# Srecharan/Leaf-Grasping-Vision-ML

Hardware: AMD Instinct MI355X
Metric: frames/sec (1080p depth+mask) grasp scoring, 1/8 MI355X; % HBM roofline (higher is better)
Workload: dtype f32; 1 GPU; 1080x1920 depth+mask, 8 score planes + valid + top-20 NMS + GraspPointCNN fp32 rescoring of 20 candidates; height=1080, width=1920, batches_in_flight=1, parallelism=frames sharded over 1 GPU(s), no collective

## Files before the change

### include/leafgrasp.h

```cpp
#ifndef LEAFGRASP_H
#define LEAFGRASP_H

#include <stdint.h>

#ifdef __cplusplus
extern "C" {
#endif

typedef struct lg_ctx* lg_handle;

typedef enum lg_status {
    LG_OK = 0,
    LG_ERR_INVALID = -1,
    LG_ERR_HIP = -2,
    LG_ERR_NOMEM = -3,
    LG_ERR_NO_MODEL = -4,
    LG_ERR_UNSUPPORTED = -5,
    LG_ERR_BUSY = -6
} lg_status;

enum {
    LG_MAP_SDF = 0,
    LG_MAP_APPROACH = 1,
    LG_MAP_FLATNESS = 2,
// ... 200 lines not shown

int lg_debug_dt_max(lg_handle h, int frame, uint32_t out[2], int32_t win[4]);
int lg_debug_dt_form(lg_handle h, int frame, int32_t form[2]);
int lg_debug_dt_search_form(lg_handle h, int32_t* algo);
int lg_dt_form_host(int forced, int n, int H, int W);
int lg_debug_orient_redo(lg_handle h, int32_t* n);
int lg_near_tile_rect(int bx0, int bx1, int by0, int by1, int H, int W, int halo, int32_t rect[4]);
int lg_stem_words_host(const uint64_t* bits, int H, int W, int WW, int bottom_start, int k, uint64_t* out);
int lg_stem_words_host_spans(const uint64_t* bits, int H, int W, int WW, int bottom_start, int n, int anchor, const int8_t* lo,
                             const int8_t* hi, int algo, uint64_t* out);
int lg_stem_plan(int k, int n, int anchor, const int8_t* lo, const int8_t* hi, int32_t* i0, int8_t span_lo[64], int8_t span_hi[64],
                 int8_t dlo[64], int8_t dhi[64]);
int lg_window_from_box(const uint32_t box[5], int H, int W, int search_mode, int32_t out[12]);
int lg_border_line_max(const int32_t* prof, int n, int lo, int len, uint32_t* out);
int lg_debug_near_tiles(lg_handle h, int32_t* off, int cap);
int lg_options_text(int which, char* buf, int cap);
int lg_debug_options(lg_handle h, char* buf, int cap);
int lg_debug_cnn_scored(lg_handle h, int64_t* patches);
int lg_debug_leaf_fallback(lg_handle h, int32_t* flags, int cap, int32_t* n_frames, int32_t* n_flagged);
int lg_debug_cnn_survivors(lg_handle h, int32_t* sub_frames, int32_t* n_sub, int32_t* counts, int32_t counts_cap,
                           int32_t* list, int32_t* slot, float* logits, int64_t cap, int64_t* n_slots);
int lg_debug_patch(lg_handle h, int64_t slot, float* out);
int lg_debug_isolation_fields(lg_handle h, int frame, uint32_t* dc_fix, uint32_t* dw_fix, uint32_t max_fix[2]);
int lg_label_aware_check(const lg_params* p, int has_labels);
int lg_norm3_host(const int32_t* dx, const int32_t* dy, int n, uint32_t* out);
int lg_dilate_words_host(const uint64_t* bits, int H, int W, int WW, int k, uint64_t* out);
int lg_debug_ws_plane_bytes(lg_handle h, int64_t bytes[LG_NUM_MAPS]);
int lg_wave_rows_on_mask(const uint64_t* bits, int H, int WW, int y, int w);

typedef struct lg_trainer lg_trainer;
// ... 46 lines not shown
```

### leaf-grasping-vision-ml_amd/_lib.py

```python
import ctypes as C
import os

_HERE = os.path.dirname(os.path.abspath(__file__))
LIB_PATH = os.environ.get("LG_LIB_PATH") or os.path.join(_HERE, "liblgrasp.so")

LG_NUM_MAPS = 8
MAP_NAMES = ("sdf_score", "approach_score", "flatness_map", "isolation_map", "distance_map",
             "accessibility_map", "stem_penalty", "traditional_score")
MAP_INDEX = {n: i for i, n in enumerate(MAP_NAMES)}

LG_OK, LG_ERR_INVALID, LG_ERR_HIP, LG_ERR_NOMEM, LG_ERR_NO_MODEL, LG_ERR_UNSUPPORTED, LG_ERR_BUSY = 0, -1, -2, -3, -4, -5, -6


class LgParams(C.Structure):
    _fields_ = [(n, C.c_double) for n in ("cx", "cy", "f")] + [(n, C.c_float) for n in (
        "w_approach", "w_sdf", "w_flat", "w_access", "sdf_w_interior", "sdf_w_align",
        "sdf_w_sdf", "optimal_distance", "access_w_dist", "access_w_dir", "flat_scale", "iso_w_close",
        "iso_w_wide", "iso_ramp_top", "iso_ramp_bottom", "min_edge_distance", "stem_valid_thresh")] + \
        [(n, C.c_int32) for n in ("stem_se", "stem_bottom_div", "top_k", "nms_min_distance",
                                  "pregrasp_clearance", "mask_is_bool", "gaussian_size", "chamfer_init_dist0", "label_aware")]


_FP = C.POINTER(C.c_float)

# ... 124 lines not shown
    "lg_debug_dt_form": (C.c_int, [_VP, C.c_int, C.POINTER(C.c_int32)]),
    "lg_debug_orient_redo": (C.c_int, [_VP, C.POINTER(C.c_int32)]),
    "lg_options_text": (C.c_int, [C.c_int, C.c_char_p, C.c_int]),
    "lg_debug_options": (C.c_int, [_VP, C.c_char_p, C.c_int]),
    "lg_debug_dt_search_form": (C.c_int, [_VP, C.POINTER(C.c_int32)]),
    "lg_dt_form_host": (C.c_int, [C.c_int, C.c_int, C.c_int, C.c_int]),
    "lg_near_tile_rect": (C.c_int, [C.c_int, C.c_int, C.c_int, C.c_int, C.c_int, C.c_int, C.c_int, C.POINTER(C.c_int32)]),
    "lg_stem_words_host": (C.c_int, [_VP, C.c_int, C.c_int, C.c_int, C.c_int, C.c_int, _VP]),
    "lg_stem_words_host_spans": (C.c_int, [_VP, C.c_int, C.c_int, C.c_int, C.c_int, C.c_int, C.c_int, C.POINTER(C.c_int8),
                                           C.POINTER(C.c_int8), C.c_int, _VP]),
    "lg_stem_plan": (C.c_int, [C.c_int, C.c_int, C.c_int, C.POINTER(C.c_int8), C.POINTER(C.c_int8), C.POINTER(C.c_int32),
                               C.POINTER(C.c_int8), C.POINTER(C.c_int8), C.POINTER(C.c_int8), C.POINTER(C.c_int8)]),
    "lg_window_from_box": (C.c_int, [C.POINTER(C.c_uint32), C.c_int, C.c_int, C.c_int, C.POINTER(C.c_int32)]),
    "lg_border_line_max": (C.c_int, [C.POINTER(C.c_int32), C.c_int, C.c_int, C.c_int, C.POINTER(C.c_uint32)]),
    "lg_debug_near_tiles":(C.c_int, [_VP, C.POINTER(C.c_int32), C.c_int]),
    "lg_debug_cnn_scored": (C.c_int, [_VP, C.POINTER(C.c_int64)]),
    "lg_debug_leaf_fallback": (C.c_int, [_VP, C.POINTER(C.c_int32), C.c_int, C.POINTER(C.c_int32), C.POINTER(C.c_int32)]),
    "lg_debug_cnn_survivors": (C.c_int, [_VP, C.POINTER(C.c_int32), C.POINTER(C.c_int32), C.POINTER(C.c_int32), C.c_int32,
                                         C.POINTER(C.c_int32), C.POINTER(C.c_int32), _FP, C.c_int64, C.POINTER(C.c_int64)]),
    "lg_debug_patch": (C.c_int, [_VP, C.c_int64, _FP]),
    "lg_debug_isolation_fields": (C.c_int, [_VP, C.c_int, _VP, _VP, C.POINTER(C.c_uint32)]),
    "lg_label_aware_check": (C.c_int, [C.POINTER(LgParams), C.c_int]),
    "lg_norm3_host": (C.c_int, [_VP, _VP, C.c_int, _VP]),
    "lg_dilate_words_host": (C.c_int, [_VP, C.c_int, C.c_int, C.c_int, C.c_int, _VP]),
    "lg_debug_ws_plane_bytes": (C.c_int, [_VP, C.POINTER(C.c_int64)]),
    "lg_wave_rows_on_mask": (C.c_int, [_VP, C.c_int, C.c_int, C.c_int, C.c_int]),
    "lg_harvest_patches": (C.c_int, [_VP, _VP, _VP, _VP, C.c_int, C.c_int, C.c_int, _VP, _VP, _VP, _VP, _VP, _VP, _VP]),
    "lg_negative_masks": (C.c_int, [_VP, _VP, _VP, C.c_int, C.c_int, _VP, _VP, _VP]),
    "lg_leaf_contour": (C.c_int, [_VP, _VP, C.c_int, C.c_int, _VP, C.c_int, C.POINTER(C.c_int), _VP]),
    "lg_train_create": (C.c_int, [C.c_int, C.c_int, C.POINTER(C.c_int32), C.c_int, C.c_int, C.POINTER(_VP)]),
# ... 58 lines not shown
```

### leaf-grasping-vision-ml_amd/csrc/lg_cnn.h

```cpp
#pragma once
#include <hip/hip_runtime.h>

#include <string>

#include "../../include/leafgrasp.h"

struct RtLayer { int cin, cout, cinp, coutp, wi; bool pool; };

struct LgCnnPlan {
    int n_layers = 6;
    RtLayer layers[8] = {};
    bool standard = true;
    int F = 256, Fp = 256, npix = 16;
    size_t act_per_patch = 64 * 32 * 32;
    int hid = 16;
    int dims[5] = {256, 256, 128, 64, 1};
};
int lg_cnn_plan(int n_blocks, const int32_t* filters, int attention_type, bool need_head, LgCnnPlan* p, std::string* err);
bool wino_supported(int cin, int cout, int wi, bool pool);
bool lg_head_supported(int F, int npix);

struct LgCnn : LgCnnPlan {
    bool loaded = false;
    float* wconv[8] = {nullptr};
// ... 14 lines not shown
    size_t act_per[8] = {0};
    float* in_halo = nullptr;
    float* zeros = nullptr;
    float* kpart = nullptr;
    unsigned* kflag = nullptr;
    unsigned* kerr_host = nullptr;
    unsigned* kerr_dev = nullptr;
    int wino_mask = 0x3f;
    int capN = 0;
    long long weight_allocs = 0;
};

int lg_cnn_upload(LgCnn* c, const lg_cnn_weights* w, std::string* err);
void lg_cnn_free(LgCnn* c);
int lg_cnn_run(LgCnn* c, const float* patches, bool haloed_in, int N, float* logits, hipStream_t s, std::string* err,
               bool allow_split = true, const int* n_dev = nullptr);
bool lg_cnn_counts_on_device(const LgCnn* c);
size_t lg_cnn_halo_patch_floats(void);
bool lg_cnn_take_error(LgCnn* c);

struct LgTrainView {
    int device = 0, n_blocks = 0, att = 0, F = 0, hid = 0;
    int filters[4] = {0, 0, 0, 0};
    float bn_eps = 1e-5f;
    const float* P = nullptr;
    const float* B = nullptr;
    size_t conv_w[8] = {0}, conv_b[8] = {0}, bn_g[8] = {0}, bn_b[8] = {0};
    size_t bn_m[8] = {0}, bn_v[8] = {0};
    size_t att_w = 0, att_b = 0, ca_w1 = 0, ca_b1 = 0, ca_w2 = 0, ca_b2 = 0;
    size_t fc_w[4] = {0}, fc_b[4] = {0}, fbn_g[3] = {0}, fbn_b[3] = {0};
    size_t fbn_m[3] = {0}, fbn_v[3] = {0};
// ... 6 lines not shown
```

### leaf-grasping-vision-ml_amd/csrc/lg_cnn.hip

```cpp
#include "lg_cnn.h"

#include <math.h>

#include <algorithm>
#include <type_traits>

typedef float f32x16 __attribute__((ext_vector_type(16)));

#ifndef LG_W4_S0
#define LG_W4_S0 9
#define LG_W4_S1 0
#define LG_W4_S2 0
#define LG_W4_S3 0
#define LG_W4_S4 3
#endif
#ifndef LG_W4_NT
#define LG_W4_NT 0
#endif
#ifndef LG_W4_EXP
#define LG_W4_EXP 0
#endif

namespace {

// ... 1163 lines not shown
        c->act_per[L] = per;
        ok = hipMalloc((void**)&c->act[L], (size_t)N * per * sizeof(float)) == hipSuccess &&
             hipMemsetAsync(c->act[L], 0, (size_t)N * per * sizeof(float), s) == hipSuccess;
    }
    ok = ok && hipMalloc((void**)&c->in_halo, (size_t)N * lg_cnn_halo_patch_floats() * sizeof(float)) == hipSuccess &&
         hipMemsetAsync(c->in_halo, 0, (size_t)N * lg_cnn_halo_patch_floats() * sizeof(float), s) == hipSuccess;
    if (!ok) {
        *err = "lg_cnn_forward: activation workspace allocation failed";
        return LG_ERR_NOMEM;
    }
    c->capN = N;
    return LG_OK;
}

static int lg_cnn_run_slice(LgCnn* c, const float* patches, bool haloed_in, int N, float* logits, hipStream_t s, std::string* err,
                            bool allow_split, const int* n_dev, int n_off);

bool lg_cnn_counts_on_device(const LgCnn* c) {
    return c->loaded && !c->use_f23 && (c->wino_mask & 1) && (!c->standard || c->wino_mask == 0x3f);
}

int lg_cnn_run(LgCnn* c, const float* patches, bool haloed_in, int N, float* logits, hipStream_t s, std::string* err,
               bool allow_split, const int* n_dev) {
    if (!c->loaded) { *err = "no model"; return LG_ERR_NO_MODEL; }
    if (n_dev && !(haloed_in && lg_cnn_counts_on_device(c))) { *err = "lg_cnn_run: no device-side patch count on this path"; return LG_ERR_UNSUPPORTED; }
    const int max_slice = 8192;
    const size_t pstride = haloed_in ? lg_cnn_halo_patch_floats() : (size_t)9 * 1024;
    for (int off = 0; off < N; off += max_slice) {
        const int n = N - off < max_slice ? N - off : max_slice;
        int rc = lg_cnn_run_slice(c, patches + (size_t)off * pstride, haloed_in, n, logits + off, s, err, allow_split, n_dev, off);
        if (rc) return rc;
    }
    return LG_OK;
}

static int lg_cnn_run_slice(LgCnn* c, const float* patches, bool haloed_in, int N, float* logits, hipStream_t s, std::string* err,
                            bool allow_split, const int* n_dev, int n_off) {
    int rc = ensure_act(c, N, s, err);
    if (rc) return rc;
    const float* x = patches;
    if (!haloed_in) {
        hipLaunchKernelGGL(lg_repack_kernel, dim3((unsigned)(N * 9)), dim3(256), 0, s, patches, c->in_halo, (long long)N * 9);
        x = c->in_halo;
    }
    if (!c->use_f23 && (c->wino_mask & 1) &&
        launch_wino4_rt(12, c->layers[0].coutp, 32, false, true, x, c->uwino4[0], c->bconv[0], c->act[0], N, c->kpart, c->kflag, c->kerr_dev, s, allow_split, n_dev, n_off)) {
    } else if (c->layers[0].coutp == 64) launch_conv0<64>(x, c, c->act[0], N, s);
    else launch_conv0<128>(x, c, c->act[0], N, s);
    const float* cur = c->act[0];
    if (c->standard) {
        const int wmask = c->wino_mask;
#define LG_LAYER(L, KC, PP, CP)                                                                                     \
    do {                                                                                                            \
        const RtLayer& l = c->layers[L];                                                                            \
        if (!(wmask & (1 << L))) launch_conv<L, KC, PP, CP>(cur, c, c->act[L], N, s);                               \
        else if (c->use_f23) launch_wino_rt(l.cinp, l.coutp, l.wi, l.pool, L != 5, cur, c->uwino[L], c->bconv[L], c->act[L], N, s); \
        else launch_wino4_rt(l.cinp, l.coutp, l.wi, l.pool, L != 5, cur, c->uwino4[L], c->bconv[L], c->act[L], N, c->kpart, c->kflag, c->kerr_dev, s, allow_split, n_dev, n_off); \
        cur = c->act[L];                                                                                            \
    } while (0)
        LG_LAYER(1, 8, 4, 1);
        LG_LAYER(2, 8, 4, 1);
        LG_LAYER(3, 8, 4, 1);
        LG_LAYER(4, 4, 1, 4);
        LG_LAYER(5, 4, 1, 4);
#undef LG_LAYER
    } else {
        for (int L = 1; L < c->n_layers; L++) {
            const RtLayer& l = c->layers[L];
            const bool okl = c->use_f23 ? launch_wino_rt(l.cinp, l.coutp, l.wi, l.pool, L + 1 < c->n_layers, cur, c->uwino[L], c->bconv[L], c->act[L], N, s)
                                        : launch_wino4_rt(l.cinp, l.coutp, l.wi, l.pool, L + 1 < c->n_layers, cur, c->uwino4[L], c->bconv[L], c->act[L], N, c->kpart, c->kflag, c->kerr_dev, s, allow_split, n_dev, n_off);
            if (!okl) {
                *err = "lg_cnn_forward: unsupported layer shape";
                return LG_ERR_UNSUPPORTED;
            }
            cur = c->act[L];
        }
    }
#define LG_HEAD(F_, NP_)                                                                                              \
    if (c->F == F_ && c->npix == NP_) {                                                                                \
        hipLaunchKernelGGL((lg_head_kernel<F_, NP_>), dim3(N), dim3(256), 0, s, cur, c->Fp, c->att_type, c->att_w, c->att_b, \
                           c->ca_w1, c->ca_b1, c->ca_w2, c->ca_b2, c->fcw[0], c->fcb[0], c->fcw[1], c->fcb[1], c->fcw[2],  \
                           c->fcb[2], c->fcw[3], c->fcb[3], logits, n_dev, n_off);                                                 \
        return LG_OK;                                                                                                  \
    }
    LG_HEAD(256, 16) LG_HEAD(128, 16) LG_HEAD(512, 16) LG_HEAD(512, 4)
#undef LG_HEAD
    *err = "lg_cnn_forward: unsupported classifier size";
    return LG_ERR_UNSUPPORTED;
}
```

### leaf-grasping-vision-ml_amd/csrc/lg_ctx.h

```cpp
#pragma once
#include <math.h>
#include <stdio.h>

#include <atomic>
#include <functional>
#include <string>
#include <vector>

#include "lg_cnn.h"
#include "lg_collect.h"
#include "lg_internal.h"
#include "lg_leaf.h"
#include "lg_midrib.h"
#include "lg_mlsel.h"
#include "lg_options.h"
#include "lg_orient.h"
#include "lg_pool.h"

struct LgProfSlot {
    std::string name;
    std::vector<hipEvent_t> ev;
    size_t used = 0;
    int launches = 0;
    double total_ms = 0.0;
};

struct lg_ctx {
    int device = 0;
    std::string err;
    hipStream_t copy_stream = nullptr;
    hipEvent_t ev_prep = nullptr, ev_copy = nullptr;
    hipStream_t s_dt[2] = {nullptr, nullptr}, s_main = nullptr, s_topk = nullptr;
    std::vector<hipEvent_t> ev_pool;
    hipEvent_t ev_begin = nullptr;
    int capB = 0, capH = 0, capW = 0, capK = 0;
    uint32_t* tmp = nullptr;
// ... 36 lines not shown
    int last_scored_subs = 0;
    int last_cnn_B = 0, last_cnn_K = 0, last_cnn_SB = 0;
    bool last_cnn_pruned = false;
    lg_grasp_result* res_dev = nullptr;
    lg_grasp_result* res_host = nullptr;
    lg_grasp_candidate* cand_rows_dev = nullptr;
    lg_grasp_candidate* cand_rows_host = nullptr;
    size_t cand_rows_cap = 0;
    LgCnn cnn;
    LgLeafWs* leaf = nullptr;
    LgLeafProf* leaf_prof = nullptr;
    LgOrientWs* orient = nullptr;
    hipEvent_t ev_orient = nullptr, ev_side = nullptr, ev_search = nullptr;
    int last_dt_algo = 0;
    int prof_on = 0;
    std::vector<LgProfSlot> prof;
    LgPool* pool = nullptr;
    LgOptions opt;
    long long last_patch_floats = 0;
    bool export_pending = false;
    std::string orient_note;
    std::atomic<bool> busy{false};
    LgMidribWs* midrib = nullptr;
    void* eval_ws = nullptr;
    size_t eval_cap = 0;
    LgMlBuffers ml = {};
    size_t ml_cap_BM = 0, ml_cap_BH = 0;
    int ml_cap_B = 0;
    float* ml_patches = nullptr;
    int ml_patches_cap = 0;
// ... 48 lines not shown
    bool ext = false;
    ProfScope(lg_ctx* h_, const char* name, hipStream_t s_, bool ext_ = false) : h(h_), s(s_), ext(ext_) {
        if (!h->prof_on || (h->prof_on == 2 && !ext)) return;
        for (auto& p : h->prof)
            if (p.name == name) slot = &p;
        if (!slot) {
            h->prof.push_back(LgProfSlot());
            slot = &h->prof.back();
            slot->name = name;
        }
        if (slot->used + 2 > slot->ev.size()) {
            hipEvent_t a, b;
            if (hipEventCreate(&a) != hipSuccess || hipEventCreate(&b) != hipSuccess) { slot = nullptr; return; }
            slot->ev.push_back(a);
            slot->ev.push_back(b);
        }
        e0 = slot->ev[slot->used];
        if (!ext) hipEventRecord(e0, s);
        e1 = slot->ev[slot->used + 1];
        slot->used += 2;
    }
    ~ProfScope() {
        if (slot && e1 && !ext) hipEventRecord(e1, s);
    }
};

inline void prof_flush(lg_ctx* h) {
    for (auto& p : h->prof) {
        for (size_t i = 0; i + 1 < p.used; i += 2) {
            float ms = 0.f;
            if (hipEventElapsedTime(&ms, p.ev[i], p.ev[i + 1]) == hipSuccess) {
                p.total_ms += ms;
                p.launches++;
            }
        }
        p.used = 0;
    }
}

template <typename T>
inline hipError_t dev_alloc(T** p, size_t n) {
    return hipMalloc((void**)p, n * sizeof(T));
}

inline void parallel_for(lg_ctx* h, int n, const std::function<void(int)>& fn) {
    if (h->pool && n > 1) h->pool->run(n, fn);
    else
        for (int i = 0; i < n; i++) fn(i);
// ... 18 lines not shown
```

### leaf-grasping-vision-ml_amd/csrc/lg_planes.h

```cpp
#pragma once
#include "lg_internal.h"

#define LG_MAX_GAUSS 15
struct LgGaussTaps { float k[LG_MAX_GAUSS]; };

__host__ __device__ inline int lg_near_tiles(int bx0, int bx1, int by0, int by1, int H, int W, int halo, int* tx_lo, int* tx_hi,
                                             int* ty_lo, int* ty_hi) {
    const int tiles_x = (W + LG_TW - 1) / LG_TW, tiles_y = (H + LG_TH - 1) / LG_TH;
    const int xa = bx0 - (LG_TW + 7), xb = bx1 + 8;
    const int ya = by0 - (LG_TH - 1 + halo), yb = by1 + LG_TH + halo;
    const int x_lo = xa > 0 ? (xa + LG_TW - 1) / LG_TW : 0, y_lo = ya > 0 ? (ya + LG_TH - 1) / LG_TH : 0;
    const int x_hi = xb < 0 ? -1 : (xb / LG_TW < tiles_x ? xb / LG_TW : tiles_x - 1);
    const int y_hi = yb < 0 ? -1 : (yb / LG_TH < tiles_y ? yb / LG_TH : tiles_y - 1);
    if (bx1 < bx0 || x_lo > x_hi || y_lo > y_hi) {
        *tx_lo = 0; *tx_hi = -1; *ty_lo = 0; *ty_hi = -1;
        return 0;
    }
    *tx_lo = x_lo; *tx_hi = x_hi; *ty_lo = y_lo; *ty_hi = y_hi;
    return (x_hi - x_lo + 1) * (y_hi - y_lo + 1);
}
__host__ __device__ inline int lg_near_tiles(const LgWin& w, int H, int W, int halo, int* tx_lo, int* tx_hi, int* ty_lo, int* ty_hi) {
    return lg_near_tiles(w.bx0, w.bx1, w.by0, w.by1, H, W, halo, tx_lo, tx_hi, ty_lo, ty_hi);
}

// ... 18 lines not shown
    float sdf_w_interior, sdf_w_align, sdf_w_sdf, optimal_distance;
    float access_w_dist, access_w_dir, flat_scale;
    float iso_w_close, iso_w_wide, iso_ramp_top, iso_ramp_bottom, iso_inv_max;
    float min_edge_distance, stem_valid_thresh;
    float inv_maxd;
    uint32_t init0;
    float inv_2s2, iso_ramp_step;
    float k1[7];
    int gauss_r;
    int no_skip;
    int nt_stores;
    int persist;
    int tpw;
    const int32_t* near_off;
    int near_total;
    int near_tpw;
};

void lg_launch_final(const LgFinalArgs& a, hipStream_t s, hipEvent_t ev_start = nullptr, hipEvent_t ev_stop = nullptr);
void lg_launch_near_tiles(const LgWin* win, int B, int H, int W, int halo, int32_t* near_off, int32_t* near_off_host_dev,
                          unsigned long long* tilekeys, uint8_t* tile_state, hipStream_t s);
void lg_launch_smooth(const float* src, float* dst, int B, int H, int W, int S, const LgGaussTaps& taps, hipStream_t s);
```

### leaf-grasping-vision-ml_amd/csrc/lg_planes.hip

```cpp
#include "lg_planes.h"
#include "lg_pixel.h"
#include "lg_wave.h"

#include <hip/hip_ext.h>

#include <algorithm>

#ifndef LG_FINAL_WPE
#define LG_FINAL_WPE 8
#endif
#define LG_FINAL_WPE_ATTR __attribute__((amdgpu_waves_per_eu(LG_FINAL_WPE, LG_FINAL_WPE)))
template <bool VEC, bool ALL, int R, bool SCORE = false>
__global__ __launch_bounds__(256) LG_FINAL_WPE_ATTR void lg_final_kernel(LgFinalArgs a_) {
    static_assert(!(ALL && SCORE), "score-only stores fewer planes than ALL");
    constexpr int HALO = R + 1;
    static_assert(R >= 0 && HALO <= 4, "the depth tile carries 4 halo columns");
    constexpr int DW = 72;
    constexpr int DH = LG_TH + 2 * HALO;
    constexpr int GW = LG_TW + 2;
    constexpr int GH = LG_TH + 2;
    __shared__ __attribute__((aligned(16))) float s_dm[DH * DW];
    __shared__ float s_h[DH * GW];
    float* const s_g = s_dm;
    static_assert(GH * (GW + 2) <= DH * DW, "g tile must fit in the depth tile");
// ... 18 lines not shown
    if (it >= it_end) return;
    int frame = __builtin_amdgcn_readfirstlane((xcd_first + it) / ntile);
    int tile = xcd_first + it - frame * ntile;
    const int step_f = __builtin_amdgcn_readfirstlane(stride / ntile), step_t = stride - step_f * ntile;
    int par = 0;
    for (; it < it_end;
         it += stride, frame += step_f, tile += step_t, frame += (tile >= ntile ? 1 : 0), tile -= (tile >= ntile ? ntile : 0)) {
    asm volatile("" : "+s"(ap));
    int t = threadIdx.x;
    asm volatile("" : "+v"(t));
    const int tiles_x = ap->tiles_x;
    const int H = ap->H, W = ap->W, WW = ap->WW;
    int li = 0;
    if (near) {
        lg_off_ptr noff = (lg_off_ptr)ap->near_off;
        li = xcd_first + it;
        int lo = 0, hi = ap->B;
        while (hi - lo > 1) {
            const int mid = (lo + hi) >> 1;
            if (noff[mid] <= li) lo = mid; else hi = mid;
        }
        frame = lo;
        li -= noff[lo];
    }
    int rx0, rx1, ry0, ry1;
    {
        const __attribute__((address_space(4))) LgWin* wp = (const __attribute__((address_space(4))) LgWin*)(ap->win + frame);
        lg_near_tiles(wp->bx0, wp->bx1, wp->by0, wp->by1, H, W, HALO, &rx0, &rx1, &ry0, &ry1);
    }
    if (near) {
        const int nx = rx1 - rx0 + 1;
// ... 457 lines not shown
```

### leaf-grasping-vision-ml_amd/csrc/lg_select.hip

```cpp
#include <string.h>

#include <algorithm>
#include <chrono>

#include "lg_ctx.h"
#include "lg_dt.h"

namespace {

void reset_last(lg_ctx* h) {
    h->last_near_B = 0; h->last_iso_B = 0;
    h->last_scored = 0; h->last_scored_subs = 0; h->last_cnn_B = 0; h->last_patch_floats = 0;
}

template <typename T>
void free_dev(T*& p) { if (p) hipFree(p); p = nullptr; }
template <typename T>
void free_pinned(T*& p) { if (p) hipHostFree(p); p = nullptr; }

template <typename T>
hipError_t regrow_dev(T** p, size_t n) {
    if (*p) hipDeviceSynchronize();
    free_dev(*p);
    const hipError_t e = dev_alloc(p, n);
    if (e != hipSuccess) (void)hipGetLastError();
    return e;
// ... 487 lines not shown
        a.init0 = (uint32_t)P.chamfer_init_dist0;
        a.iso_inv_max = 1.0f / mx;
    }
    a.min_edge_distance = P.min_edge_distance; a.stem_valid_thresh = P.stem_valid_thresh;
    a.inv_maxd = (float)(1.0 / sqrt((double)W * W + (double)H * H));
    a.inv_2s2 = 1.0f / (2.0f * P.optimal_distance * P.optimal_distance);
    a.iso_ramp_step = (H > 1) ? (P.iso_ramp_bottom - P.iso_ramp_top) / (float)(H - 1) : 0.0f;
    gaussian1d(P.gaussian_size, a.k1);
    a.gauss_r = P.gaussian_size / 2;
    a.no_skip = h->opt.no_skip;
    a.persist = h->opt.final_persist;
    a.tpw = h->opt.final_tpw;
    a.nt_stores = 0;
    if (pl.near) {
        LG_HIP(h, hipEventSynchronize(h->ev_near));
        a.near_off = h->near_off;
        a.near_total = h->near_off_host[n];
        a.near_tpw = h->opt.final_near;
    }
    {
        ProfScope ps(h, "final", s, true);
        lg_launch_final(a, s, ps.slot ? ps.e0 : nullptr, ps.slot ? ps.e1 : nullptr);
    }
    if (keep) *keep = a;
    return LG_OK;
}

int make_plan(lg_ctx* h, Plan& pl, const float* depth, const uint8_t* mask, int B, int H, int W, const lg_params* pin,
              float* const out_maps[LG_NUM_MAPS], uint8_t* out_valid) {
    if (!depth || !mask || B <= 0 || H < 8 || W < 8 || W > 8192 || H > 16384)
        return fail(h, LG_ERR_INVALID, "bad pointer or shape (need H,W >= 8, W <= 8192)");
    if (pin) pl.P = *pin; else lg_default_params(&pl.P);
// ... 35 lines not shown
    void host(int i) { if (on) t[i] = now(); }
    void mark(int i) { if (gpu) hipEventRecord(ev[i], s); }
    void print(int B) {
        if (!on) return;
        if (gpu) {
            float a[5] = {0};
            for (int i = 1; i <= 4; i++) hipEventElapsedTime(&a[i], ev[START], ev[i]);
            fprintf(stderr, "[lg] gpu timeline (ms since call start): sweeps done %.3f | planes %.3f | topk %.3f | cnn %.3f\n", a[1], a[2],
                    a[3], a[4]);
        }
        fprintf(stderr, "[lg] B=%d enq1 %.3f | wait bits %.3f | orient %.3f | enq2 %.3f | gpu wait %.3f | post %.3f ms\n", B,
                t[ENQ1] - t[START], 0.0, t[ORIENT] - t[ENQ1], t[ENQ2] - t[ORIENT], t[SYNC] - t[ENQ2], now() - t[SYNC]);
    }
};

template <typename AfterPrep>
int enq_front(lg_ctx* h, Plan& pl, hipStream_t s, LgFinalArgs* fargs, Timeline* tl, AfterPrep&& after_prep) {
    pl.near = pl.sparse && h->opt.final_near > 0 && h->opt.subbatch == 0 && h->opt.no_skip == 0;
    int rc = enq_prep(h, pl, 0, pl.B, s, h->ev_prep);
    if (rc) return rc;
    if ((rc = after_prep())) return rc;
    if ((rc = enq_dt(h, pl, 0, pl.B, s))) return rc;
    if ((rc = enq_iso(h, pl, s))) return rc;
    if (tl) { tl->mark(Timeline::SWEEPS); tl->host(Timeline::ENQ1); }
    bool upload_fp = true;
    if ((rc = finish_orient(h, pl, 0, pl.B, &upload_fp))) return rc;
    if (tl) tl->host(Timeline::ORIENT);
    if ((rc = enq_final(h, pl, 0, pl.B, s, upload_fp, fargs))) return rc;
    enq_iso_plane(h, pl, *fargs, s);
    return LG_OK;
}
int nothing_after_prep() { return LG_OK; }

LgFinishArgs finish_args(lg_ctx* h, const Plan& pl, int K, bool use_cnn) {
    LgFinishArgs fa;
    memset(&fa, 0, sizeof(fa));
    fa.bits2 = pl.label_aware ? h->iso_others : nullptr;
    fa.fp = h->fp_dev; fa.bits = h->bits; fa.out = h->res_host_dev ? h->res_host_dev : h->res_dev;
    fa.B = pl.B; fa.H = pl.H; fa.W = pl.W; fa.WW = pl.WW; fa.K = K; fa.use_cnn = use_cnn ? 1 : 0; fa.mask_is_bool = pl.P.mask_is_bool;
    fa.cx = pl.P.cx; fa.cy = pl.P.cy; fa.f = pl.P.f;
    lg_make_se_spans(2 * pl.P.pregrasp_clearance + 1, &fa.se);
    return fa;
// ... 35 lines not shown
    reset_last(h);
    if (pl.label_aware) rc = ensure_iso_ws(h, pl, "lg_select_grasp_labels: label-aware workspace");
    if (!rc && cands) rc = ensure_cand_rows(h, (size_t)B * P.top_k);
    if (rc) return rc;
    const bool use_cnn = h->cnn.loaded;
    const bool prune = use_cnn && !cands && h->opt.cnn_prune && lg_cnn_counts_on_device(&h->cnn);
    if (use_cnn) h->last_scored = (long long)B * P.top_k;
    pl.defer = pl.sparse && h->opt.defer_planes;
    if ((rc = take_planes(h, pl, use_cnn))) return rc;
    const int K = P.top_k;
    const size_t px = (size_t)H * W;
    const int tiles = pl.tiles_x * pl.tiles_y;

    int SB = B;
    if (h->opt.subbatch > 0 && !pl.label_aware) SB = h->opt.subbatch;
    const int nsub = (B + SB - 1) / SB;
    const bool piped = nsub > 1;
    std::vector<LgFinalArgs> fargs((size_t)nsub);
    hipStream_t sD[2] = {piped ? h->s_dt[0] : s, piped ? h->s_dt[1] : s};
    hipStream_t sM = piped ? h->s_main : s, sT = piped ? h->s_topk : s;
    while ((int)h->ev_pool.size() < 6 * nsub) {
        hipEvent_t e;
        LG_HIP(h, hipEventCreateWithFlags(&e, hipEventDisableTiming));
        h->ev_pool.push_back(e);
    }
    auto EV = [&](int k, int which) { return h->ev_pool[6 * k + which]; };
    const LgIsoFields iso = iso_fields(h);
    auto enq_T = [&](int k) {
        const int off = k * SB, n = std::min(SB, B - off);
        ProfScope ps(h, "topk", sT);
        lg_launch_topk(pl.maps[LG_MAP_TRADITIONAL] + off * px, pl.valid + off * px, depth + off * px,
                       h->tilekeys + (size_t)off * tiles, pl.sparse ? h->tile_state + (size_t)off * tiles : nullptr,
                       P.flat_scale, P.w_flat, true, n, H, W, K, P.nms_min_distance,
                       h->cand_xy + (size_t)off * K * 2, h->cand_n + off, h->cand_info + (size_t)off * K * 2, sT,
                       prune ? h->surv_keep + off : nullptr, P.mask_is_bool);
    };
    auto enq_G = [&](int k) -> int {
        const int off = k * SB, n = std::min(SB, B - off);
        if (piped) LG_HIP(h, hipStreamWaitEvent(sM, EV(k, 4), 0));
        if (use_cnn) {
            const int32_t* list = prune ? h->surv_list + (size_t)off * K : nullptr;
            const int32_t* count = prune ? h->surv_count + k : nullptr;
            if (prune) {
                ProfScope ps(h, "survivors", sM);
                lg_launch_survivors(h->surv_keep + off, n, K, h->surv_list + (size_t)off * K, h->surv_slot + (size_t)off * K,
                                    h->surv_count + k, sM);
            }
            {
                ProfScope ps(h, "gather", sM);
                const float* mp[LG_NUM_MAPS];
                for (int i = 0; i < LG_NUM_MAPS; i++) mp[i] = pl.maps[i] ? pl.maps[i] + off * px : nullptr;
                lg_launch_gather(depth + off * px, mask + off * px, mp, pl.sparse ? h->tile_state + (size_t)off * tiles : nullptr,
                                 P.flat_scale, n, H, W, K, h->cand_xy + (size_t)off * K * 2,
                                 h->cand_n + off, h->patches + (size_t)off * K * lg_cnn_halo_patch_floats(), true, sM, list, count,
                                 pl.defer ? &fargs[k] : nullptr, pl.label_aware ? &iso : nullptr);
            }
            std::string err;
            {
                ProfScope ps(h, "cnn", sM);
                int r2 = lg_cnn_run(&h->cnn, h->patches + (size_t)off * K * lg_cnn_halo_patch_floats(), true, n * K, h->logits + (size_t)off * K, sM, &err,
                                    false, count);
                if (r2) return fail(h, r2, err.c_str());
            }
        }
        return LG_OK;
    };
    Timeline tl(h->opt.trace, !piped, s);
    if (!piped) {
        if ((rc = enq_front(h, pl, s, &fargs[0], &tl, nothing_after_prep))) return rc;
        tl.mark(Timeline::PLANES);
        enq_T(0);
        tl.mark(Timeline::TOPK);
    } else {
        LG_HIP(h, hipEventRecord(h->ev_begin, s));
        for (hipStream_t q : {sD[0], sD[1], sM, sT}) LG_HIP(h, hipStreamWaitEvent(q, h->ev_begin, 0));
        if ((rc = enq_prep(h, pl, 0, B, sD[0], h->ev_prep))) return rc;
        LG_HIP(h, hipStreamWaitEvent(sD[1], h->ev_prep, 0));
        for (int k = 0; k < nsub; k++) {
            const int off = k * SB, n = std::min(SB, B - off);
            if ((rc = enq_dt(h, pl, off, n, sD[k & 1]))) return rc;
            LG_HIP(h, hipEventRecord(EV(k, 2), sD[k & 1]));
        }
        tl.host(Timeline::ENQ1);
        bool upload_fp = true;
        if ((rc = finish_orient(h, pl, 0, B, &upload_fp))) return rc;
        tl.host(Timeline::ORIENT);
        for (int k = 0; k < nsub; k++) {
            const int off = k * SB, n = std::min(SB, B - off);
            LG_HIP(h, hipStreamWaitEvent(sM, EV(k, 2), 0));
            if ((rc = enq_final(h, pl, off, n, sM, upload_fp, &fargs[k]))) return rc;
            LG_HIP(h, hipEventRecord(EV(k, 3), sM));
            LG_HIP(h, hipStreamWaitEvent(sT, EV(k, 3), 0));
            enq_T(k);
            LG_HIP(h, hipEventRecord(EV(k, 4), sT));
            if (k >= 1) { rc = enq_G(k - 1); if (rc) return rc; }
        }
    }
    if ((rc = enq_G(nsub - 1))) return rc;
    if (prune) h->last_scored_subs = nsub;
    tl.mark(Timeline::CNN);
    if (piped) {
        for (hipStream_t q : {sD[0], sD[1], sM, sT}) {
            LG_HIP(h, hipEventRecord(EV(0, 5), q));
            LG_HIP(h, hipStreamWaitEvent(s, EV(0, 5), 0));
            LG_HIP(h, hipStreamSynchronize(q));
        }
    }
    {
        LgFinishArgs fa = finish_args(h, pl, K, use_cnn);
        fa.cand_n = h->cand_n; fa.cand_xy = h->cand_xy; fa.cand_info = h->cand_info; fa.logits = h->logits;
        fa.slot = prune ? h->surv_slot : nullptr; fa.slot_frames = SB;
        {
            ProfScope ps(h, "finish", s);
// ... 198 lines not shown
    }
    LgFinishArgs fa = finish_args(h, ps, 1, false);
    fa.cand_n = c.pick.n; fa.cand_xy = c.pick.xy; fa.cand_info = c.pick.info; fa.slot_frames = B;
    {
        ProfScope pf(h, "finish", s);
        lg_launch_finish(fa, s);
    }
    lg_launch_col_rows(c.pick, fa.out, B, s);
    return return_results(h, ps, results, false, "lg_select_grasp_collect", s);
}

}

extern "C" {

int lg_score_maps(lg_handle h, const float* depth, const uint8_t* mask, int B, int H, int W, const lg_params* pin,
                  float* const out_maps[LG_NUM_MAPS], uint8_t* out_valid, float* theta_host, void* stream_) {
    if (!h) return LG_ERR_INVALID;
    LG_ENTER(h);
    Plan pl;
    int rc = make_plan(h, pl, depth, mask, B, H, W, pin, out_maps, out_valid);
    if (rc) return rc;
    if (lg_label_aware_check(&pl.P, 0)) return fail(h, LG_ERR_INVALID, "lg_score_maps: label_aware needs the label image (lg_select_grasp_labels, lg_select_grasp_candidates_labels)");
    hipStream_t s = (hipStream_t)stream_;
    LG_HIP(h, hipSetDevice(h->device));
    if ((rc = ensure_ws(h, B, H, W, pl.P.top_k))) return rc;
    if ((rc = take_planes(h, pl, false))) return rc;
    LgFinalArgs fargs;
    if ((rc = enq_front(h, pl, s, &fargs, nullptr, nothing_after_prep))) return rc;
    if (theta_host)
// ... 153 lines not shown
```

### leaf-grasping-vision-ml_amd/grasp_point_selector.py

```python
import ctypes as C
import math
import os
import threading

import numpy as np
import torch

from . import _lib
from ._lib import LG_NUM_MAPS, MAP_NAMES, LgGraspCandidate, LgGraspResult, LgMlSample, LgMlSampling, LgParams, check, lib
from ._log import logerr, loginfo, logwarn
from .cnn import pack_state_dict
from .image_processor import flatness_config

_RESULT_DTYPE = np.dtype([(n, np.int32 if t is C.c_int else np.float32) for n, t in LgGraspResult._fields_])
assert _RESULT_DTYPE.itemsize == C.sizeof(LgGraspResult)
GRASP_CANDIDATE_DTYPE = np.dtype([(n, np.int32 if t is C.c_int32 else np.float32) for n, t in LgGraspCandidate._fields_])
assert GRASP_CANDIDATE_DTYPE.itemsize == C.sizeof(LgGraspCandidate)
_ML_FIELDS = ("ml_score", "ml_confidence", "combined")
ML_SAMPLE_DTYPE = np.dtype([(n, np.int32 if t is C.c_int32 else np.float32) for n, t in LgMlSample._fields_])
assert ML_SAMPLE_DTYPE.itemsize == C.sizeof(LgMlSample) == 20

_VP = C.c_void_p

MIDRIB_FOUND, MIDRIB_NO_CONTOUR, MIDRIB_THIN, MIDRIB_TOO_FEW = 0, 1, 2, 3
# ... 215 lines not shown
        i32 = C.POINTER(C.c_int32)
        rc = lib.lg_debug_cnn_survivors(self._h, C.byref(sub_frames), C.byref(n_sub), None, 0, None, None, None, 0,
                                        C.byref(n_slots))
        if rc != 0:
            raise RuntimeError(lib.lg_last_error(self._h).decode())
        n = int(n_slots.value)
        counts = np.zeros(int(n_sub.value), np.int32)
        lst, slot, logits = np.zeros(n, np.int32), np.zeros(n, np.int32), np.zeros(n, np.float32)
        rc = lib.lg_debug_cnn_survivors(self._h, C.byref(sub_frames), C.byref(n_sub), counts.ctypes.data_as(i32), counts.size,
                                        lst.ctypes.data_as(i32), slot.ctypes.data_as(i32),
                                        logits.ctypes.data_as(C.POINTER(C.c_float)), n, C.byref(n_slots))
        if rc != 0:
            raise RuntimeError(lib.lg_last_error(self._h).decode())
        return dict(sub_frames=int(sub_frames.value), n_sub=int(n_sub.value), counts=counts, list=lst, slot=slot, logits=logits)

    def patch(self, slot):
        out = np.zeros((9, 32, 32), np.float32)
        rc = lib.lg_debug_patch(self._h, int(slot), out.ctypes.data_as(C.POINTER(C.c_float)))
        if rc != 0:
            raise RuntimeError(lib.lg_last_error(self._h).decode())
        return out

    def isolation_fields(self, frame, H, W):
        dc, dw = np.zeros((H, W), np.uint32), np.zeros((H, W), np.uint32)
        mx = (C.c_uint32 * 2)()
        rc = lib.lg_debug_isolation_fields(self._h, int(frame), dc.ctypes.data, dw.ctypes.data, mx)
        if rc < 0:
            raise RuntimeError(lib.lg_last_error(self._h).decode())
        return (dc, dw, (int(mx[0]), int(mx[1]))) if rc == 1 else None

# ... 403 lines not shown
```

Measured before the change: 132,800 frames/s.

## Split final-plane, top-k and CNN tail into parallel stream lanes

After the shared front sweeps (prep, distance transform, isolation, orient), the batch is split into up to four sub-batches. Each sub-batch gets its own stream for the final plane pass, top-k/NMS and CNN rescoring. Each lane writes to its own offset in the CNN activation buffer, and near-tile offsets are rebased per slice. The aim is to overlap the tail stages of different sub-batches and keep the GPU busier for mid-sized batches. In exchange it adds cross-stream events, larger reserved activation memory and a process-wide in-flight counter, and it only engages automatically for large enough batches that fit in one CNN slice.

```diff
diff --git a/include/leafgrasp.h b/include/leafgrasp.h
--- a/include/leafgrasp.h
+++ b/include/leafgrasp.h
@@ -238,6 +238,8 @@
 int lg_window_from_box(const uint32_t box[5], int H, int W, int search_mode, int32_t out[12]);
 int lg_border_line_max(const int32_t* prof, int n, int lo, int len, uint32_t* out);
 int lg_debug_near_tiles(lg_handle h, int32_t* off, int cap);
+int lg_tail_lane_plan(int B, int requested, int eligible, int32_t* lanes, int32_t* sb);
+int lg_debug_tail_lanes(lg_handle h, int set, int32_t* last);
 int lg_options_text(int which, char* buf, int cap);
 int lg_debug_options(lg_handle h, char* buf, int cap);
 int lg_debug_cnn_scored(lg_handle h, int64_t* patches);
diff --git a/leaf-grasping-vision-ml_amd/_lib.py b/leaf-grasping-vision-ml_amd/_lib.py
--- a/leaf-grasping-vision-ml_amd/_lib.py
+++ b/leaf-grasping-vision-ml_amd/_lib.py
@@ -162,6 +162,8 @@
     "lg_window_from_box": (C.c_int, [C.POINTER(C.c_uint32), C.c_int, C.c_int, C.c_int, C.POINTER(C.c_int32)]),
     "lg_border_line_max": (C.c_int, [C.POINTER(C.c_int32), C.c_int, C.c_int, C.c_int, C.POINTER(C.c_uint32)]),
     "lg_debug_near_tiles":(C.c_int, [_VP, C.POINTER(C.c_int32), C.c_int]),
+    "lg_tail_lane_plan": (C.c_int, [C.c_int, C.c_int, C.c_int, C.POINTER(C.c_int32), C.POINTER(C.c_int32)]),
+    "lg_debug_tail_lanes": (C.c_int, [_VP, C.c_int, C.POINTER(C.c_int32)]),
     "lg_debug_cnn_scored": (C.c_int, [_VP, C.POINTER(C.c_int64)]),
     "lg_debug_leaf_fallback": (C.c_int, [_VP, C.POINTER(C.c_int32), C.c_int, C.POINTER(C.c_int32), C.POINTER(C.c_int32)]),
     "lg_debug_cnn_survivors": (C.c_int, [_VP, C.POINTER(C.c_int32), C.POINTER(C.c_int32), C.POINTER(C.c_int32), C.c_int32,
diff --git a/leaf-grasping-vision-ml_amd/csrc/lg_cnn.h b/leaf-grasping-vision-ml_amd/csrc/lg_cnn.h
--- a/leaf-grasping-vision-ml_amd/csrc/lg_cnn.h
+++ b/leaf-grasping-vision-ml_amd/csrc/lg_cnn.h
@@ -52,7 +52,9 @@
 int lg_cnn_upload(LgCnn* c, const lg_cnn_weights* w, std::string* err);
 void lg_cnn_free(LgCnn* c);
 int lg_cnn_run(LgCnn* c, const float* patches, bool haloed_in, int N, float* logits, hipStream_t s, std::string* err,
-               bool allow_split = true, const int* n_dev = nullptr);
+               bool allow_split = true, const int* n_dev = nullptr, int act_off = 0);
+int lg_cnn_act_slots(int N);
+int lg_cnn_reserve(LgCnn* c, int slots, hipStream_t s, std::string* err);
 bool lg_cnn_counts_on_device(const LgCnn* c);
 size_t lg_cnn_halo_patch_floats(void);
 bool lg_cnn_take_error(LgCnn* c);
diff --git a/leaf-grasping-vision-ml_amd/csrc/lg_cnn.hip b/leaf-grasping-vision-ml_amd/csrc/lg_cnn.hip
--- a/leaf-grasping-vision-ml_amd/csrc/lg_cnn.hip
+++ b/leaf-grasping-vision-ml_amd/csrc/lg_cnn.hip
@@ -1201,49 +1201,59 @@
 }
 
 static int lg_cnn_run_slice(LgCnn* c, const float* patches, bool haloed_in, int N, float* logits, hipStream_t s, std::string* err,
-                            bool allow_split, const int* n_dev, int n_off);
+                            bool allow_split, const int* n_dev, int n_off, int act_off);
 
 bool lg_cnn_counts_on_device(const LgCnn* c) {
     return c->loaded && !c->use_f23 && (c->wino_mask & 1) && (!c->standard || c->wino_mask == 0x3f);
 }
 
+constexpr int LG_CNN_MAX_SLICE = 8192;
+int lg_cnn_act_slots(int N) { return N < LG_CNN_MAX_SLICE ? N : LG_CNN_MAX_SLICE; }
+int lg_cnn_reserve(LgCnn* c, int slots, hipStream_t s, std::string* err) {
+    if (!c->loaded) { *err = "no model"; return LG_ERR_NO_MODEL; }
+    return ensure_act(c, slots, s, err);
+}
+
 int lg_cnn_run(LgCnn* c, const float* patches, bool haloed_in, int N, float* logits, hipStream_t s, std::string* err,
-               bool allow_split, const int* n_dev) {
+               bool allow_split, const int* n_dev, int act_off) {
     if (!c->loaded) { *err = "no model"; return LG_ERR_NO_MODEL; }
     if (n_dev && !(haloed_in && lg_cnn_counts_on_device(c))) { *err = "lg_cnn_run: no device-side patch count on this path"; return LG_ERR_UNSUPPORTED; }
-    const int max_slice = 8192;
+    if (act_off && !haloed_in) { *err = "lg_cnn_run: an activation offset needs haloed patches"; return LG_ERR_UNSUPPORTED; }
+    const int max_slice = LG_CNN_MAX_SLICE;
     const size_t pstride = haloed_in ? lg_cnn_halo_patch_floats() : (size_t)9 * 1024;
     for (int off = 0; off < N; off += max_slice) {
         const int n = N - off < max_slice ? N - off : max_slice;
-        int rc = lg_cnn_run_slice(c, patches + (size_t)off * pstride, haloed_in, n, logits + off, s, err, allow_split, n_dev, off);
+        int rc = lg_cnn_run_slice(c, patches + (size_t)off * pstride, haloed_in, n, logits + off, s, err, allow_split, n_dev, off, act_off);
         if (rc) return rc;
     }
     return LG_OK;
 }
 
 static int lg_cnn_run_slice(LgCnn* c, const float* patches, bool haloed_in, int N, float* logits, hipStream_t s, std::string* err,
-                            bool allow_split, const int* n_dev, int n_off) {
-    int rc = ensure_act(c, N, s, err);
+                            bool allow_split, const int* n_dev, int n_off, int act_off) {
+    int rc = ensure_act(c, act_off + N, s, err);
     if (rc) return rc;
+    float* act[8];
+    for (int L = 0; L < c->n_layers; L++) act[L] = c->act[L] + (size_t)act_off * c->act_per[L];
     const float* x = patches;
     if (!haloed_in) {
         hipLaunchKernelGGL(lg_repack_kernel, dim3((unsigned)(N * 9)), dim3(256), 0, s, patches, c->in_halo, (long long)N * 9);
         x = c->in_halo;
     }
     if (!c->use_f23 && (c->wino_mask & 1) &&
-        launch_wino4_rt(12, c->layers[0].coutp, 32, false, true, x, c->uwino4[0], c->bconv[0], c->act[0], N, c->kpart, c->kflag, c->kerr_dev, s, allow_split, n_dev, n_off)) {
-    } else if (c->layers[0].coutp == 64) launch_conv0<64>(x, c, c->act[0], N, s);
-    else launch_conv0<128>(x, c, c->act[0], N, s);
-    const float* cur = c->act[0];
+        launch_wino4_rt(12, c->layers[0].coutp, 32, false, true, x, c->uwino4[0], c->bconv[0], act[0], N, c->kpart, c->kflag, c->kerr_dev, s, allow_split, n_dev, n_off)) {
+    } else if (c->layers[0].coutp == 64) launch_conv0<64>(x, c, act[0], N, s);
+    else launch_conv0<128>(x, c, act[0], N, s);
+    const float* cur = act[0];
     if (c->standard) {
         const int wmask = c->wino_mask;
 #define LG_LAYER(L, KC, PP, CP)                                                                                     \
     do {                                                                                                            \
         const RtLayer& l = c->layers[L];                                                                            \
-        if (!(wmask & (1 << L))) launch_conv<L, KC, PP, CP>(cur, c, c->act[L], N, s);                               \
-        else if (c->use_f23) launch_wino_rt(l.cinp, l.coutp, l.wi, l.pool, L != 5, cur, c->uwino[L], c->bconv[L], c->act[L], N, s); \
-        else launch_wino4_rt(l.cinp, l.coutp, l.wi, l.pool, L != 5, cur, c->uwino4[L], c->bconv[L], c->act[L], N, c->kpart, c->kflag, c->kerr_dev, s, allow_split, n_dev, n_off); \
-        cur = c->act[L];                                                                                            \
+        if (!(wmask & (1 << L))) launch_conv<L, KC, PP, CP>(cur, c, act[L], N, s);                               \
+        else if (c->use_f23) launch_wino_rt(l.cinp, l.coutp, l.wi, l.pool, L != 5, cur, c->uwino[L], c->bconv[L], act[L], N, s); \
+        else launch_wino4_rt(l.cinp, l.coutp, l.wi, l.pool, L != 5, cur, c->uwino4[L], c->bconv[L], act[L], N, c->kpart, c->kflag, c->kerr_dev, s, allow_split, n_dev, n_off); \
+        cur = act[L];                                                                                            \
     } while (0)
         LG_LAYER(1, 8, 4, 1);
         LG_LAYER(2, 8, 4, 1);
@@ -1254,13 +1264,13 @@
     } else {
         for (int L = 1; L < c->n_layers; L++) {
             const RtLayer& l = c->layers[L];
-            const bool okl = c->use_f23 ? launch_wino_rt(l.cinp, l.coutp, l.wi, l.pool, L + 1 < c->n_layers, cur, c->uwino[L], c->bconv[L], c->act[L], N, s)
-                                        : launch_wino4_rt(l.cinp, l.coutp, l.wi, l.pool, L + 1 < c->n_layers, cur, c->uwino4[L], c->bconv[L], c->act[L], N, c->kpart, c->kflag, c->kerr_dev, s, allow_split, n_dev, n_off);
+            const bool okl = c->use_f23 ? launch_wino_rt(l.cinp, l.coutp, l.wi, l.pool, L + 1 < c->n_layers, cur, c->uwino[L], c->bconv[L], act[L], N, s)
+                                        : launch_wino4_rt(l.cinp, l.coutp, l.wi, l.pool, L + 1 < c->n_layers, cur, c->uwino4[L], c->bconv[L], act[L], N, c->kpart, c->kflag, c->kerr_dev, s, allow_split, n_dev, n_off);
             if (!okl) {
                 *err = "lg_cnn_forward: unsupported layer shape";
                 return LG_ERR_UNSUPPORTED;
             }
-            cur = c->act[L];
+            cur = act[L];
         }
     }
 #define LG_HEAD(F_, NP_)                                                                                              \
diff --git a/leaf-grasping-vision-ml_amd/csrc/lg_ctx.h b/leaf-grasping-vision-ml_amd/csrc/lg_ctx.h
--- a/leaf-grasping-vision-ml_amd/csrc/lg_ctx.h
+++ b/leaf-grasping-vision-ml_amd/csrc/lg_ctx.h
@@ -20,6 +20,7 @@
 struct LgProfSlot {
     std::string name;
     std::vector<hipEvent_t> ev;
+    std::vector<uint8_t> cont;
     size_t used = 0;
     int launches = 0;
     double total_ms = 0.0;
@@ -86,6 +87,8 @@
     hipEvent_t ev_orient = nullptr, ev_side = nullptr, ev_search = nullptr;
     int last_dt_algo = 0;
     int prof_on = 0;
+    bool prof_cont = false;
+    int tail_lanes_req = 0, last_tail_lanes = 0;
     std::vector<LgProfSlot> prof;
     LgPool* pool = nullptr;
     LgOptions opt;
@@ -164,7 +167,9 @@
             if (hipEventCreate(&a) != hipSuccess || hipEventCreate(&b) != hipSuccess) { slot = nullptr; return; }
             slot->ev.push_back(a);
             slot->ev.push_back(b);
+            slot->cont.push_back(0);
         }
+        slot->cont[slot->used / 2] = h->prof_cont ? 1 : 0;
         e0 = slot->ev[slot->used];
         if (!ext) hipEventRecord(e0, s);
         e1 = slot->ev[slot->used + 1];
@@ -181,7 +186,7 @@
             float ms = 0.f;
             if (hipEventElapsedTime(&ms, p.ev[i], p.ev[i + 1]) == hipSuccess) {
                 p.total_ms += ms;
-                p.launches++;
+                if (!p.cont[i / 2]) p.launches++;
             }
         }
         p.used = 0;
diff --git a/leaf-grasping-vision-ml_amd/csrc/lg_planes.h b/leaf-grasping-vision-ml_amd/csrc/lg_planes.h
--- a/leaf-grasping-vision-ml_amd/csrc/lg_planes.h
+++ b/leaf-grasping-vision-ml_amd/csrc/lg_planes.h
@@ -56,6 +56,7 @@
     int tpw;
     const int32_t* near_off;
     int near_total;
+    int near_base;
     int near_tpw;
 };
 
diff --git a/leaf-grasping-vision-ml_amd/csrc/lg_planes.hip b/leaf-grasping-vision-ml_amd/csrc/lg_planes.hip
--- a/leaf-grasping-vision-ml_amd/csrc/lg_planes.hip
+++ b/leaf-grasping-vision-ml_amd/csrc/lg_planes.hip
@@ -56,7 +56,7 @@
     int li = 0;
     if (near) {
         lg_off_ptr noff = (lg_off_ptr)ap->near_off;
-        li = xcd_first + it;
+        li = ap->near_base + xcd_first + it;
         int lo = 0, hi = ap->B;
         while (hi - lo > 1) {
             const int mid = (lo + hi) >> 1;
diff --git a/leaf-grasping-vision-ml_amd/csrc/lg_select.hip b/leaf-grasping-vision-ml_amd/csrc/lg_select.hip
--- a/leaf-grasping-vision-ml_amd/csrc/lg_select.hip
+++ b/leaf-grasping-vision-ml_amd/csrc/lg_select.hip
@@ -6,10 +6,23 @@
 #include "lg_ctx.h"
 #include "lg_dt.h"
 
+#ifndef LG_TAIL_LANES_AUTO
+#define LG_TAIL_LANES_AUTO 2
+#endif
+#ifndef LG_TAIL_LANES_MIN_B
+#define LG_TAIL_LANES_MIN_B 256
+#endif
+#ifndef LG_TAIL_LANE_STREAMS
+#define LG_TAIL_LANE_STREAMS h->s_main, h->s_topk, h->s_dt[0]
+#endif
+
 namespace {
+
+std::atomic<int> g_select_in_flight{0};
 
 void reset_last(lg_ctx* h) {
     h->last_near_B = 0; h->last_iso_B = 0;
+    h->last_tail_lanes = 0;
     h->last_scored = 0; h->last_scored_subs = 0; h->last_cnn_B = 0; h->last_patch_floats = 0;
 }
 
@@ -527,8 +540,9 @@
     a.nt_stores = 0;
     if (pl.near) {
         LG_HIP(h, hipEventSynchronize(h->ev_near));
-        a.near_off = h->near_off;
-        a.near_total = h->near_off_host[n];
+        a.near_off = h->near_off + off;
+        a.near_base = h->near_off_host[off];
+        a.near_total = h->near_off_host[off + n] - h->near_off_host[off];
         a.near_tpw = h->opt.final_near;
     }
     {
@@ -594,18 +608,30 @@
     }
 };
 
+bool takes_near_launch(const lg_ctx* h, const Plan& pl) {
+    return pl.sparse && h->opt.final_near > 0 && h->opt.subbatch == 0 && h->opt.no_skip == 0;
+}
+
 template <typename AfterPrep>
-int enq_front(lg_ctx* h, Plan& pl, hipStream_t s, LgFinalArgs* fargs, Timeline* tl, AfterPrep&& after_prep) {
-    pl.near = pl.sparse && h->opt.final_near > 0 && h->opt.subbatch == 0 && h->opt.no_skip == 0;
+int enq_front_sweeps(lg_ctx* h, Plan& pl, hipStream_t s, Timeline* tl, AfterPrep&& after_prep, bool* upload_fp) {
+    pl.near = takes_near_launch(h, pl);
     int rc = enq_prep(h, pl, 0, pl.B, s, h->ev_prep);
     if (rc) return rc;
     if ((rc = after_prep())) return rc;
     if ((rc = enq_dt(h, pl, 0, pl.B, s))) return rc;
     if ((rc = enq_iso(h, pl, s))) return rc;
     if (tl) { tl->mark(Timeline::SWEEPS); tl->host(Timeline::ENQ1); }
+    *upload_fp = true;
+    if ((rc = finish_orient(h, pl, 0, pl.B, upload_fp))) return rc;
+    if (tl) tl->host(Timeline::ORIENT);
+    return LG_OK;
+}
+
+template <typename AfterPrep>
+int enq_front(lg_ctx* h, Plan& pl, hipStream_t s, LgFinalArgs* fargs, Timeline* tl, AfterPrep&& after_prep) {
     bool upload_fp = true;
-    if ((rc = finish_orient(h, pl, 0, pl.B, &upload_fp))) return rc;
-    if (tl) tl->host(Timeline::ORIENT);
+    int rc = enq_front_sweeps(h, pl, s, tl, after_prep, &upload_fp);
+    if (rc) return rc;
     if ((rc = enq_final(h, pl, 0, pl.B, s, upload_fp, fargs))) return rc;
     enq_iso_plane(h, pl, *fargs, s);
     return LG_OK;
@@ -671,8 +697,27 @@
 
     int SB = B;
     if (h->opt.subbatch > 0 && !pl.label_aware) SB = h->opt.subbatch;
+    const bool piped = SB < B;
+    struct InFlight {
+        const int others;
+        InFlight() : others(g_select_in_flight.fetch_add(1, std::memory_order_relaxed)) {}
+        ~InFlight() { g_select_in_flight.fetch_sub(1, std::memory_order_relaxed); }
+    } in_flight;
+    const bool one_slice = lg_cnn_act_slots(B * K) == B * K;
+    const int lanes_req = h->tail_lanes_req ? h->tail_lanes_req : (in_flight.others || !one_slice ? 1 : 0);
+    int32_t lanes = 1, lane_sb = B;
+    lg_tail_lane_plan(B, lanes_req, !piped && prune && !pl.label_aware && takes_near_launch(h, pl), &lanes, &lane_sb);
+    const bool laned = lanes > 1;
+    if (laned) SB = lane_sb;
     const int nsub = (B + SB - 1) / SB;
-    const bool piped = nsub > 1;
+    h->last_tail_lanes = laned ? nsub : 1;
+    const int lane_slots = lg_cnn_act_slots(SB * K);
+    if (laned) {
+        std::string err;
+        const int r2 = lg_cnn_reserve(&h->cnn, (nsub - 1) * lane_slots + lg_cnn_act_slots((B - (nsub - 1) * SB) * K), s, &err);
+        if (r2) return fail(h, r2, err.c_str());
+    }
+    struct ContGuard { lg_ctx* h; ~ContGuard() { h->prof_cont = false; } } cont_guard{h};
     std::vector<LgFinalArgs> fargs((size_t)nsub);
     hipStream_t sD[2] = {piped ? h->s_dt[0] : s, piped ? h->s_dt[1] : s};
     hipStream_t sM = piped ? h->s_main : s, sT = piped ? h->s_topk : s;
@@ -692,7 +737,7 @@
                        h->cand_xy + (size_t)off * K * 2, h->cand_n + off, h->cand_info + (size_t)off * K * 2, sT,
                        prune ? h->surv_keep + off : nullptr, P.mask_is_bool);
     };
-    auto enq_G = [&](int k) -> int {
+    auto enq_G = [&](int k, int act_off = 0) -> int {
         const int off = k * SB, n = std::min(SB, B - off);
         if (piped) LG_HIP(h, hipStreamWaitEvent(sM, EV(k, 4), 0));
         if (use_cnn) {
@@ -716,14 +761,33 @@
             {
                 ProfScope ps(h, "cnn", sM);
                 int r2 = lg_cnn_run(&h->cnn, h->patches + (size_t)off * K * lg_cnn_halo_patch_floats(), true, n * K, h->logits + (size_t)off * K, sM, &err,
-                                    false, count);
+                                    false, count, act_off);
                 if (r2) return fail(h, r2, err.c_str());
             }
         }
         return LG_OK;
     };
     Timeline tl(h->opt.trace, !piped, s);
-    if (!piped) {
+    if (laned) {
+        bool upload_fp = true;
+        if ((rc = enq_front_sweeps(h, pl, s, &tl, nothing_after_prep, &upload_fp))) return rc;
+        const hipStream_t lane_s[4] = {s, LG_TAIL_LANE_STREAMS};
+        for (int k = 0; k < nsub; k++) {
+            const int off = k * SB, n = std::min(SB, B - off);
+            sM = sT = lane_s[k];
+            h->prof_cont = k > 0;
+            if (k) LG_HIP(h, hipStreamWaitEvent(sM, EV(k - 1, 3), 0));
+            if ((rc = enq_final(h, pl, off, n, sM, upload_fp, &fargs[k]))) return rc;
+            if (k + 1 < nsub) LG_HIP(h, hipEventRecord(EV(k, 3), sM));
+            if (!k) tl.mark(Timeline::PLANES);
+            enq_T(k);
+            if (!k) tl.mark(Timeline::TOPK);
+            if ((rc = enq_G(k, k * lane_slots))) return rc;
+            if (k) LG_HIP(h, hipEventRecord(EV(k, 5), sM));
+        }
+        h->prof_cont = false;
+        for (int k = 1; k < nsub; k++) LG_HIP(h, hipStreamWaitEvent(s, EV(k, 5), 0));
+    } else if (!piped) {
         if ((rc = enq_front(h, pl, s, &fargs[0], &tl, nothing_after_prep))) return rc;
         tl.mark(Timeline::PLANES);
         enq_T(0);
@@ -753,7 +817,7 @@
             if (k >= 1) { rc = enq_G(k - 1); if (rc) return rc; }
         }
     }
-    if ((rc = enq_G(nsub - 1))) return rc;
+    if (!laned && (rc = enq_G(nsub - 1))) return rc;
     if (prune) h->last_scored_subs = nsub;
     tl.mark(Timeline::CNN);
     if (piped) {
@@ -982,6 +1046,24 @@
 
 extern "C" {
 
+int lg_tail_lane_plan(int B, int requested, int eligible, int32_t* lanes, int32_t* sb) {
+    if (B < 1 || requested < 0 || requested > 4 || !lanes || !sb) return LG_ERR_INVALID;
+    int want = requested ? requested : (B >= LG_TAIL_LANES_MIN_B ? LG_TAIL_LANES_AUTO : 1);
+    if (!eligible) want = 1;
+    want = std::min(want, B);
+    *sb = (B + want - 1) / want;
+    *lanes = (B + *sb - 1) / *sb;
+    return LG_OK;
+}
+
+int lg_debug_tail_lanes(lg_handle h, int set, int32_t* last) {
+    if (!h || set > 4) return LG_ERR_INVALID;
+    LG_ENTER(h);
+    if (set >= 0) h->tail_lanes_req = set;
+    if (last) *last = h->last_tail_lanes;
+    return LG_OK;
+}
+
 int lg_score_maps(lg_handle h, const float* depth, const uint8_t* mask, int B, int H, int W, const lg_params* pin,
                   float* const out_maps[LG_NUM_MAPS], uint8_t* out_valid, float* theta_host, void* stream_) {
     if (!h) return LG_ERR_INVALID;
diff --git a/leaf-grasping-vision-ml_amd/grasp_point_selector.py b/leaf-grasping-vision-ml_amd/grasp_point_selector.py
--- a/leaf-grasping-vision-ml_amd/grasp_point_selector.py
+++ b/leaf-grasping-vision-ml_amd/grasp_point_selector.py
@@ -253,6 +253,13 @@
             raise RuntimeError(lib.lg_last_error(self._h).decode())
         return dict(sub_frames=int(sub_frames.value), n_sub=int(n_sub.value), counts=counts, list=lst, slot=slot, logits=logits)
 
+    def tail_lanes(self, lanes=None):
+        last = C.c_int32()
+        rc = lib.lg_debug_tail_lanes(self._h, -1 if lanes is None else int(lanes), C.byref(last))
+        if rc != 0:
+            raise RuntimeError(f"lg_debug_tail_lanes({lanes}) -> {rc}")
+        return int(last.value)
+
     def patch(self, slot):
         out = np.zeros((9, 32, 32), np.float32)
         rc = lib.lg_debug_patch(self._h, int(slot), out.ctypes.data_as(C.POINTER(C.c_float)))
```

New measurement: 137,800 frames/s, median of 6. +3.8%, better.
